# jones-lab-tamu/CBAS

Measured on AMD Instinct MI355X. Metric: frames/sec DINOv3-B/16 224px encode+LSTM classify, 1/2/4/8 MI355X, higher is better.
Workload: dtype f16; 1 GPU; DINOv3 ViT-B/16 66624-frame synthetic 224x224 RGB clip per GPU, batch=64, chunked encode + BiLSTM head (C=9, seq_len=31); batch=64, batches_in_flight=2, frames_per_gpu=66624, parallelism=clip-per-gpu x1, weights=synthetic (seeded counter-based generator), operands=fp16 MFMA, fp32 accumulate/residual; head fp32

## Files before the change

cbas_amd/csrc/gemm_epilogue.h:

```cpp
#pragma once
#include "kernels.h"

__device__ __forceinline__ f32x4 rope_rot(f32x4 a, f32x4 c, f32x4 b, f32x4 s) {
    f32x4 t;
    {
#pragma clang fp contract(off)
        t = b * s;
    }
    return __builtin_elementwise_fma(a, c, t);
}

typedef float f32x2 __attribute__((ext_vector_type(2)));
constexpr int LN_BLOCK = 256;
__device__ __forceinline__ float row16_sum(float v) {
    v += dpp_f32<0xB1>(v);
    v += dpp_f32<0x4E>(v);
    v += dpp_f32<0x141>(v);
    v += dpp_f32<0x140>(v);
    return v;
}
template <int NB>
__device__ __forceinline__ f32x2 ln_pool(const f32x2 (&b)[NB], int nb, float n) {
    float s = 0.f, q = 0.f;
#pragma unroll
    for (int k = 0; k < NB; ++k)
        if (k < nb) { s += b[k][0]; q += b[k][1]; }
    const float mean = s / ((float)nb * n);
    float between = 0.f;
#pragma unroll
    for (int k = 0; k < NB; ++k)
        if (k < nb) {
            const float d = b[k][0] * (1.0f / n) - mean;
            between = fmaf(d, d, between);
// ... 49 lines not shown
            const int n = ncol + j * 16;
            const f32x4 bv = *reinterpret_cast<const f32x4*>(p.bias + n);
            const f32x4 lv = *reinterpret_cast<const f32x4*>(p.lambda + n);
            float* xp = p.out_f32 + (size_t)m * p.ldo + n;
            const f32x4 xv = *reinterpret_cast<const f32x4*>(xp);
            *reinterpret_cast<f32x4*>(xp) = (acc[j] + bv) * lv + xv;
        }
    } else if (EPI == EPI_SWIGLU) {
#pragma unroll
        for (int j = 0; j < 2; ++j) {
            const int n = ncol + j * 16;
            const f32x4 gv = swiglu_fast4(acc[j] + *reinterpret_cast<const f32x4*>(p.bias + n),
                                          acc[j + 2] + *reinterpret_cast<const f32x4*>(p.bias + n + 32));
            const f16x4 hv = {(f16)gv[0], (f16)gv[1], (f16)gv[2], (f16)gv[3]};
            *reinterpret_cast<f16x4*>(p.out_f16 + (size_t)m * p.ldo + (head_col0 >> 1) + (lane >> 4) * 4 + j * 16) = hv;
        }
    } else {
#pragma unroll
        for (int j = 0; j < 4; ++j) {
            const int n = ncol + j * 16;
            const f32x4 bv = *reinterpret_cast<const f32x4*>(p.bias + n);
            const f32x4 w = acc[j] + bv;
            const f32x4 gv = gelu_fast4(w);
            const f16x4 hv = {(f16)gv[0], (f16)gv[1], (f16)gv[2], (f16)gv[3]};
            *reinterpret_cast<f16x4*>(p.out_f16 + (size_t)m * p.ldo + n) = hv;
        }
    }
}

#ifndef CBAS_EPI_PASS_SLABS
#define CBAS_EPI_PASS_SLABS 1
#endif
struct NoPrefetch { __device__ __forceinline__ void operator()() const {} };

template <int EPIX, int TM, typename Pre = NoPrefetch>
__device__ __forceinline__ void gemm_epilogue_tile(const GemmParams& p, int row_base, int head_col0, int lane,
                                                   const f32x4 (&acc)[TM][4], char* scratch, Pre pre = Pre(),
                                                   const float* rope_lds = nullptr, f32x2* ln_red = nullptr) {
    constexpr int EPI = epi_base(EPIX);
    constexpr bool LN = EPIX != EPI;
    const int li = lane & 15, g = lane >> 4;
    if (EPI == EPI_PATCH) {
        pre();
#pragma unroll
        for (int i = 0; i < TM; ++i) {
            const int m = row_base + i * 16 + li;
            if (m < p.M) gemm_epilogue_row<EPI_PATCH>(p, m, head_col0, lane, acc[i]);
        }
    } else if (EPI == EPI_RESID) {
        const f32x4 bvt = *reinterpret_cast<const f32x4*>(p.bias + head_col0 + li * 4);
        const f32x4 lvt = *reinterpret_cast<const f32x4*>(p.lambda + head_col0 + li * 4);
        f32x4 xs[2][4];
        auto load_x = [&](int i, f32x4 (&dst)[4]) {
#pragma unroll
            for (int it = 0; it < 4; ++it) {
                int m = row_base + i * 16 + it * 4 + g;
                m = m < p.M ? m : p.M - 1;
                dst[it] = *reinterpret_cast<const f32x4*>(p.out_f32 + (size_t)m * p.ldo + head_col0 + li * 4);
            }
        };
        load_x(0, xs[0]);
        if (TM > 1) load_x(1, xs[1]);
        pre();
#pragma unroll
        for (int i = 0; i < TM; ++i) {
            char* sc = scratch + (i & 1) * 4096;
#pragma unroll
            for (int j = 0; j < 4; ++j) {
                const int q = (4 * j + g) ^ li;
                *reinterpret_cast<f32x4*>(sc + li * 256 + q * 16) = acc[i][j];
            }
            asm volatile("" ::: "memory");
            uint2 h16r[4];
#pragma unroll
            for (int it = 0; it < 4; ++it) {
                const int r = it * 4 + g;
                const f32x4 y = *reinterpret_cast<const f32x4*>(sc + r * 256 + ((li ^ r) << 4));
                const int m = row_base + i * 16 + r;
                const f32x4 xn = (y + bvt) * lvt + xs[i & 1][it];
                if (m < p.M) *reinterpret_cast<f32x4*>(p.out_f32 + (size_t)m * p.ldo + head_col0 + li * 4) = xn;
                if (LN) {
                    const float bs = row16_sum((xn[0] + xn[1]) + (xn[2] + xn[3]));
                    const f32x4 d = xn - bs * (1.0f / 64.0f);
                    const float bq = row16_sum((d[0] * d[0] + d[1] * d[1]) + (d[2] * d[2] + d[3] * d[3]));
                    if (li == 0) ln_red[(i * 16 + r) * 4] = f32x2{bs, bq};
                    const f32x4 c = __builtin_elementwise_max(__builtin_elementwise_min(xn, f32x4{65504.f, 65504.f, 65504.f, 65504.f}),
                                                              f32x4{-65504.f, -65504.f, -65504.f, -65504.f});
                    union { f16x4 h; uint2 u; } cv;
                    cv.h = f16x4{(f16)c[0], (f16)c[1], (f16)c[2], (f16)c[3]};
                    h16r[it] = cv.u;
                }
            }
            if (LN) {
                const bool odd = li & 1;
#pragma unroll
                for (int it = 0; it < 4; it += 2) {
                    const uint2 send = odd ? h16r[it] : h16r[it + 1];
                    uint2 recv;
                    recv.x = (unsigned)__builtin_amdgcn_update_dpp(0, (int)send.x, 0xB1, 0xf, 0xf, true);
                    recv.y = (unsigned)__builtin_amdgcn_update_dpp(0, (int)send.y, 0xB1, 0xf, 0xf, true);
                    const uint2 own = odd ? h16r[it + 1] : h16r[it];
                    const uint4 outv = odd ? uint4{recv.x, recv.y, own.x, own.y} : uint4{own.x, own.y, recv.x, recv.y};
                    const int m = row_base + i * 16 + (it + (odd ? 1 : 0)) * 4 + g;
                    if (m < p.M) *reinterpret_cast<uint4*>(p.x16_out + (size_t)m * p.N + head_col0 + (li & ~1) * 4) = outv;
                }
            }
            if (i + 2 < TM) load_x(i + 2, xs[i & 1]);
            asm volatile("" ::: "memory");
        }
    } else if (EPI == EPI_GELU_F8) {
        f32x4 bv[4];
#pragma unroll
        for (int j = 0; j < 4; ++j) bv[j] = *reinterpret_cast<const f32x4*>(p.bias + head_col0 + j * 16 + g * 4);
        pre();
        uint8_t* const sc_bytes = reinterpret_cast<uint8_t*>(p.out_sc) + (size_t)(head_col0 >> 7) * p.sc_ldo * 4 + ((head_col0 & 127) >> 5);
#pragma unroll
        for (int half = 0; half < (TM + 3) / 4; ++half) {
#pragma unroll
            for (int ii = 0; ii < 4; ++ii) {
                const int i = half * 4 + ii;
                if (i >= TM) break;
                f32x4 v[4];
#pragma unroll
                for (int j = 0; j < 4; ++j) {
                    const f32x4 w = acc[i][j] + bv[j];
                    v[j] = gelu_fast4(w);
                    if (EPIX == EPI_GELU_F8_H) {
                        const f16x4 hv = {(f16)v[j][0], (f16)v[j][1], (f16)v[j][2], (f16)v[j][3]};
                        v[j] = f32x4{(float)hv[0], (float)hv[1], (float)hv[2], (float)hv[3]};
                    }
                }
                int sb[2];
#pragma unroll
                for (int b = 0; b < 2; ++b) {
                    float a = 0.f;
#pragma unroll
                    for (int e = 0; e < 4; ++e) a = fmaxf(a, fmaxf(fabsf(v[2 * b][e]), fabsf(v[2 * b + 1][e])));
                    a = xor16_max(a);
                    a = xor32_max(a);
                    sb[b] = mx_scale_byte(a);
                }
// ... 156 lines not shown
```

cbas_amd/csrc/gemm_f16_8ph.hip:

```cpp
#include <stdlib.h>
#include <map>
#include <mutex>
#include <queue>
#include <type_traits>
#include <vector>
#include "gemm_epilogue.h"
#include "vit32_epilogue.h"

namespace {

constexpr int BK = 64;
constexpr int BN = 256;

struct PPGrid {
    int main_blocks;
    int tail_row0;
    int n_tiles;
};

__device__ __forceinline__ f16x8 read_frag8(const char* lds_tile, int off) {
    return *reinterpret_cast<const f16x8*>(lds_tile + off);
}

template <int TA, int TB>
// ... 98 lines not shown
        }
    };

    int a_off[2], b_off[2];
    int sa_off = 0, sb_off = 0;
    auto set_frag_offsets = [&] {
        const int frow = lane & 15, fchunk = lane >> 4;
#pragma unroll
        for (int kk = 0; kk < 2; ++kk) {
            const int sw = ((kk * 4 + fchunk) ^ ((frow >> 1) & 7)) << 4;
            a_off[kk] = (wr * WROWS + frow) * 128 + sw;
            b_off[kk] = A_BYTES + (wc * 64 + frow) * 128 + sw;
        }
        sa_off = (wr * WROWS + frow) * 4 + fchunk;
        sb_off = 1024 + (wc * 64 + frow) * 4 + fchunk;
    };

    constexpr bool LNC = EPI == EPI_QKV_LN || EPI == EPI_GELU_LN;
    f32x2 lnp[4];
    auto load_lnp = [&] {
        if constexpr (LNC) {
            if (tid < BM) {
                int m = row0 + tid;
                m = m < p.M ? m : p.M - 1;
                const f32x2* src = reinterpret_cast<const f32x2*>(p.ln_in) + m;
#pragma unroll
                for (int k = 0; k < 4; ++k)
                    if (k < p.ln_parts) lnp[k] = src[(size_t)k * p.ln_ld];
            }
        }
    };

    f32x4 acc[TM][4];
    unsigned long long t_start = 0, t_top = 0, t_pro = 0, t_loop = 0, r_pro = 0, r_loop = 0;
    if (p.stamps) t_start = __builtin_amdgcn_s_memtime();
    load_lnp();
    stage(0, 0, 0); stage(0, 0, 1); stage(0, 0, 2); stage(0, 0, 3);

    struct Frag { f16x8 h[2]; i32x8 v; int sc; };
    Frag a[TMAX], b0[2], b1[2];

#define CBAS_SEG_BARRIER()                      \
    do {                                        \
        __builtin_amdgcn_sched_barrier(0);      \
        __builtin_amdgcn_s_barrier();           \
        __builtin_amdgcn_sched_barrier(0);      \
    } while (0)

    auto mfma_quadrant = [&](auto ha_c, Frag (&bf)[2], int hb) {
        constexpr int ha = decltype(ha_c)::value;
        constexpr int T = ha ? TB : TA, I0 = ha ? TA : 0;
        asm volatile("s_waitcnt lgkmcnt(0)" ::: "memory");
        __builtin_amdgcn_sched_barrier(0);
        __builtin_amdgcn_s_setprio(1);
        if constexpr (F8) {
#pragma unroll
            for (int i = 0; i < T; ++i)
#pragma unroll
                for (int j = 0; j < 2; ++j)
                    acc[I0 + i][hb * 2 + j] = __builtin_amdgcn_mfma_scale_f32_16x16x128_f8f6f4(
                        bf[j].v, a[i].v, acc[I0 + i][hb * 2 + j], 0, 0, 0, bf[j].sc, 0, a[i].sc);
#pragma unroll
            for (int i = 0; i < T; ++i)
#pragma unroll
                for (int j = 0; j < 2; ++j) asm volatile("" : "+v"(acc[I0 + i][hb * 2 + j]));
        } else if constexpr (SPLIT) {
// ... 12 lines not shown
                for (int i = 0; i < T; ++i)
#pragma unroll
                    for (int j = 0; j < 2; ++j)
                        acc[I0 + i][hb * 2 + j] =
                            __builtin_amdgcn_mfma_f32_16x16x32_f16(bf[j].h[kk], a[i].h[kk], acc[I0 + i][hb * 2 + j], 0, 0, 0);
        }
        __builtin_amdgcn_s_setprio(0);
    };
    auto read_frag = [&](Frag& f, const char* buf, int off0, int off1, const char* scb, int sc_off) {
        if constexpr (F8) {
            const i32x4 lo = *reinterpret_cast<const i32x4*>(buf + off0), hi = *reinterpret_cast<const i32x4*>(buf + off1);
            f.v = __builtin_shufflevector(lo, hi, 0, 1, 2, 3, 4, 5, 6, 7);
            asm volatile("ds_read_u8 %0, %1" : "=v"(f.sc) : "v"((unsigned)(uintptr_t)LDS_PTR(scb + sc_off)));
        } else {
            f.h[0] = read_frag8(buf, off0);
            f.h[1] = read_frag8(buf, off1);
        }
    };
    auto read_a = [&](const char* buf, const char* scb, auto h_c) {
        constexpr int h = decltype(h_c)::value;
        constexpr int T = h ? TB : TA, I0 = h ? TA : 0;
#pragma unroll
        for (int i = 0; i < T; ++i)
            read_frag(a[i], buf, a_off[0] + (I0 + i) * 2048, a_off[1] + (I0 + i) * 2048, scb, sa_off + (I0 + i) * 64);
    };
    auto read_b = [&](const char* buf, const char* scb, int h, Frag (&bf)[2]) {
#pragma unroll
        for (int j = 0; j < 2; ++j)
            read_frag(bf[j], buf, b_off[0] + (h * 2 + j) * 2048, b_off[1] + (h * 2 + j) * 2048, scb, sb_off + (h * 2 + j) * 64);
    };
    using H0 = std::integral_constant<int, 0>;
    using H1 = std::integral_constant<int, 1>;

    auto ktile = [&](int b, int t) {
        const char* buf = smem + b * BUF_BYTES;
        const char* scb = sc_lds + b * 2048;
        read_b(buf, scb, 0, b0);
        __builtin_amdgcn_sched_barrier(0);
        read_a(buf, scb, H0{});
        if (t + 1 < nk) stage(b ^ 1, t + 1, 3);
        if (TA == 4) { if (F8) asm volatile("s_waitcnt lgkmcnt(12)" ::: "memory"); else asm volatile("s_waitcnt lgkmcnt(8)" ::: "memory"); }
        else if (TA == 3) { if (F8) asm volatile("s_waitcnt lgkmcnt(9)" ::: "memory"); else asm volatile("s_waitcnt lgkmcnt(6)" ::: "memory"); }
        else { if (F8) asm volatile("s_waitcnt lgkmcnt(6)" ::: "memory"); else asm volatile("s_waitcnt lgkmcnt(4)" ::: "memory"); }
        CBAS_SEG_BARRIER();
        mfma_quadrant(H0{}, b0, 0);
        CBAS_SEG_BARRIER();
        read_b(buf, scb, 1, b1);
        if (t + 2 < nk) stage(b, t + 2, 0);
        CBAS_SEG_BARRIER();
        mfma_quadrant(H0{}, b1, 1);
        CBAS_SEG_BARRIER();
        read_a(buf, scb, H1{});
        if (t + 2 < nk) stage(b, t + 2, 1);
        CBAS_SEG_BARRIER();
        mfma_quadrant(H1{}, b1, 1);
        CBAS_SEG_BARRIER();
        if (t + 2 < nk) {
            stage(b, t + 2, 2);
            asm volatile("s_waitcnt vmcnt(6)" ::: "memory");
        } else {
            asm volatile("s_waitcnt vmcnt(0)" ::: "memory");
        }
        CBAS_SEG_BARRIER();
        mfma_quadrant(H1{}, b0, 0);
        CBAS_SEG_BARRIER();
    };

    for (int id = first;;) {
        if (p.stamps) t_top = __builtin_amdgcn_s_memtime();
        asm volatile("" : "+v"(lane));
        set_tile(id);
        set_frag_offsets();
#pragma unroll
        for (int i = 0; i < TM; ++i)
#pragma unroll
            for (int j = 0; j < 4; ++j) acc[i][j] = f32x4{0.f, 0.f, 0.f, 0.f};
        stage(1, 1, 0); stage(1, 1, 1); stage(1, 1, 2);
        asm volatile("s_waitcnt vmcnt(6)" ::: "memory");
        __builtin_amdgcn_s_barrier();
        if constexpr (LNC) {
            if (tid < BM) {
                const f32x2 st = ln_pool<4>(lnp, p.ln_parts, (float)LN_BLOCK);
                const float inv_d = 1.0f / (float)(p.ln_parts * LN_BLOCK);
                reinterpret_cast<f32x2*>(ln_lds)[tid] = f32x2{st[0] * inv_d, 1.0f / sqrtf(st[1] * inv_d + p.ln_eps)};
            }
        }
        if (p.stamps) { t_pro = __builtin_amdgcn_s_memtime(); r_pro = __builtin_amdgcn_s_memrealtime(); }
        if (wr == 1) __builtin_amdgcn_s_barrier();

        for (int t = 0; t < nk; t += 2) {
            ktile(0, t);
            ktile(1, t + 1);
        }
        if (wr == 0) __builtin_amdgcn_s_barrier();

        if (p.stamps) { t_loop = __builtin_amdgcn_s_memtime(); r_loop = __builtin_amdgcn_s_memrealtime(); }
        const int erow = row0 + wr * WROWS, ecol = col0 + wc * 64;
        const int next = id + stride;
        const bool has_next = next < n_kind;
        asm volatile("" : "+v"(lane));
        if (has_next) set_tile(next);
        if constexpr (SPLIT) {
            vit32_epilogue_tile<EPI, TM>(sp, erow, ecol, lane, acc, smem + BUF_BYTES + wave * 8192, [&] {
                if (has_next) { stage(0, 0, 0); stage(0, 0, 1); stage(0, 0, 2); stage(0, 0, 3); }
            }, rope_lds);
        } else
        gemm_epilogue_tile<EPI, TM>(p, erow, ecol, lane, acc, smem + BUF_BYTES + wave * 8192, [&] {
            if (has_next) { load_lnp(); stage(0, 0, 0); stage(0, 0, 1); stage(0, 0, 2); stage(0, 0, 3); }
        }, rope_lds, EPI == EPI_RESID_LN ? reinterpret_cast<f32x2*>(ln_lds) + (wr * WROWS) * 4 + wc
                                         : reinterpret_cast<f32x2*>(ln_lds) + wr * WROWS);
        if constexpr (EPI == EPI_RESID_LN) {
            asm volatile("s_waitcnt lgkmcnt(0)" ::: "memory");
            __builtin_amdgcn_s_barrier();
            if (tid < BM) {
                const f32x2* e = reinterpret_cast<const f32x2*>(ln_lds) + tid * 4;
                const f32x2 blk[4] = {e[0], e[1], e[2], e[3]};
                const int m = erow - wr * WROWS + tid;
                if (m < p.M) reinterpret_cast<f32x2*>(p.ln_out)[(size_t)((ecol - wc * 64) / LN_BLOCK) * p.ln_ld + m] = ln_pool<4>(blk, 4, 64.0f);
            }
        }
        if (p.stamps && id == first && tid == 0) {
            asm volatile("s_waitcnt vmcnt(0)" ::: "memory");
            unsigned long long* o = p.stamps + (size_t)blockIdx.x * 4;
            o[0] = t_start; o[1] = t_pro; o[2] = t_loop; o[3] = __builtin_amdgcn_s_memtime();
            p.stamps[(size_t)GEMM_STAMP_BLOCKS * 4 + blockIdx.x] = r_loop - r_pro;
        }
        if (p.stamps && id != first && !has_next && tid == 0) {
            unsigned long long* o = p.stamps + (size_t)GEMM_STAMP_BLOCKS * 5 + (size_t)blockIdx.x * 4;
            o[0] = t_top; o[1] = t_pro; o[2] = t_loop; o[3] = __builtin_amdgcn_s_memtime();
        }
        if (!has_next) break;
        id = next;
        if constexpr (EPI != EPI_RESID_LN) {
            asm volatile("s_waitcnt lgkmcnt(0)" ::: "memory");
            __builtin_amdgcn_s_barrier();
        }
    }
#undef CBAS_SEG_BARRIER
}

template <int EPI, int TA, int TB, int TAIL, bool F8>
__global__ __launch_bounds__(512, 2) void gemm_f16_8ph_kernel(GemmParams p, PPGrid g) {
    extern __shared__ __attribute__((aligned(16))) char smem[];
// ... 272 lines not shown
```

cbas_amd/csrc/vit_kernels.hip:

```cpp
#include <stdlib.h>
#include "kernels.h"

namespace {

__global__ void im2col_u8_kernel(const uint8_t* __restrict__ frames, int n, int height, int width,
                                 int64_t frame_stride, int64_t row_stride, int64_t pixel_stride,
                                 f16* __restrict__ A, int nh, int nw, int ps) {
    const int64_t gid = (int64_t)blockIdx.x * blockDim.x + threadIdx.x;
    const int64_t total = (int64_t)n * nh * ps * nw;
    if (gid >= total) return;
    const int px = gid % nw;
    const int64_t t1 = gid / nw;
    const int y = t1 % (nh * ps);
    const int b = t1 / (nh * ps);
    const int py = y / ps, i = y - py * ps;
    const uint8_t* src = frames + b * frame_stride + (int64_t)y * row_stride + (int64_t)px * ps * pixel_stride;
    f16x8 lo, hi;
#pragma unroll
    for (int j = 0; j < 8; ++j) {
        lo[j] = (f16)(float)src[j * pixel_stride];
        hi[j] = (j + 8 < ps) ? (f16)(float)src[(j + 8) * pixel_stride] : (f16)0.f;
    }
    f16* dst = A + ((int64_t)b * nh * nw + (int64_t)py * nw + px) * 256 + i * 16;
    *reinterpret_cast<f16x8*>(dst) = lo;
    *reinterpret_cast<f16x8*>(dst + 8) = hi;
}

__global__ void im2col_f32_kernel(const float* __restrict__ frames, int n, int height, int width,
                                  f16* __restrict__ A, int nh, int nw, int ps) {
    const int64_t gid = (int64_t)blockIdx.x * blockDim.x + threadIdx.x;
    const int64_t total = (int64_t)n * nh * ps * nw;
    if (gid >= total) return;
// ... 203 lines not shown
}

__device__ __forceinline__ int k_off(int row, int chunk) { return row * 128 + ((chunk ^ ((row >> 1) & 7)) << 4); }
__device__ __forceinline__ int v_off(int row, int col) {
    return row * 128 + ((((col >> 4) ^ ((row >> 1) & 3))) << 5) + ((col & 15) << 1);
}

__device__ __forceinline__ void attn_store_f8(const f32x4 (&o)[4], float inv, uint8_t* out8, uint32_t* out_sc, int sc_ld,
                                              size_t row, bool valid, int D, int hd, int g) {
    int sb[2];
#pragma unroll
    for (int b = 0; b < 2; ++b) {
        float a = 0.f;
#pragma unroll
        for (int dt = 2 * b; dt < 2 * b + 2; ++dt)
#pragma unroll
            for (int r = 0; r < 4; ++r) a = fmaxf(a, fabsf(o[dt][r] * inv));
        a = xor16_max(a);
        a = xor32_max(a);
        sb[b] = mx_scale_byte(a);
    }
    if (!valid) return;
    uint8_t* orow = out8 + row * D + hd * 64 + 4 * g;
#pragma unroll
    for (int dt = 0; dt < 4; ++dt) {
        const float m = inv * mx_inv_scale(sb[dt >> 1]);
        *reinterpret_cast<unsigned*>(orow + 16 * dt) = cvt4_e4m3(o[dt][0] * m, o[dt][1] * m, o[dt][2] * m, o[dt][3] * m);
    }
    if (g == 0)
        *reinterpret_cast<uint16_t*>(reinterpret_cast<uint8_t*>(out_sc) + ((size_t)(hd >> 1) * sc_ld + row) * 4 + (hd & 1) * 2) =
            (uint16_t)(sb[0] | (sb[1] << 8));
}

template <int NKT, int NV, int SPLIT>
#ifndef CBAS_ATTN_MIN_WAVES
#define CBAS_ATTN_MIN_WAVES 4
#endif
__global__ __launch_bounds__(SPLIT == 2 ? 256 : 512, (SPLIT == 2 ? (NKT > 14 ? 2 : 3) : (NKT > 14 ? 2 : CBAS_ATTN_MIN_WAVES)))
void attention_kernel(const f16* __restrict__ qkv, const f16* __restrict__ q_cls, void* __restrict__ out_v,
                      uint32_t* __restrict__ out_sc, int sc_ld, int T, int D, int n_heads, int n_pairs) {
    f16* __restrict__ out = reinterpret_cast<f16*>(out_v);
    extern __shared__ __attribute__((aligned(16))) char smem[];
    constexpr int NQK = NV ? NV : NKT;
    constexpr int NG = NV ? (NV + 1) / 2 : NKT / 2;
    constexpr int ROWS = NQK * 16;
    char* Vs = smem;
    char* Ks = smem + ROWS * 128;

    const int tid = threadIdx.x, lane = tid & 63, wave = tid >> 6, nwaves = blockDim.x >> 6;
    int pair = blockIdx.x, half = 0;
    if (SPLIT == 2) {
        pair = ((int)blockIdx.x >> 4) * 8 + ((int)blockIdx.x & 7);
        half = ((int)blockIdx.x >> 3) & 1;
        if (pair >= n_pairs) return;
    }
    const int b = pair / n_heads, hd = pair - b * n_heads;
    const size_t ld = (size_t)3 * D;
    const f16* qbase = qkv + (size_t)b * T * ld + hd * 64;
    const f16* kbase = qbase + D;
    const f16* vbase = qbase + 2 * D;
    const int g = lane >> 4, li = lane & 15;
    const int nq = q_cls ? 1 : T;
    const f16* qsrc = q_cls ? q_cls + (size_t)b * D + hd * 64 : qbase;
    const size_t qld = q_cls ? 0 : ld;
    const int nqt_all = (nq + 15) >> 4;
    const int q_per = SPLIT == 2 ? (nqt_all + 1) / 2 : nqt_all;
    const int qt0 = half * q_per;
    const int nqt = qt0 + q_per < nqt_all ? qt0 + q_per : nqt_all;

    auto load_q = [&](int qt, f16x8 (&qf)[2]) {
        const int q = qt * 16 + li;
        const int qrow = q < nq ? q : nq - 1;
        qf[0] = *reinterpret_cast<const f16x8*>(qsrc + (size_t)qrow * qld + g * 8);
        qf[1] = *reinterpret_cast<const f16x8*>(qsrc + (size_t)qrow * qld + 32 + g * 8);
    };
    f16x8 qf[2] = {};
    int qt = qt0 + wave;
    if (qt < nqt) load_q(qt, qf);

    {
        const int pr = lane >> 3, pos = lane & 7;
        for (int p = wave; p < ROWS / 8; p += nwaves) {
            const int r = p * 8 + pr;
            const int rs = r < T ? r : T - 1;
            const int kc = pos ^ ((r >> 1) & 7);
            const int vc = (((pos >> 1) ^ ((r >> 1) & 3)) << 1) | (pos & 1);
            __builtin_amdgcn_global_load_lds(GLB_PTR(kbase + (size_t)rs * ld + kc * 8), LDS_PTR(Ks + p * 1024), 16, 0, 0);
            __builtin_amdgcn_global_load_lds(GLB_PTR(vbase + (size_t)rs * ld + vc * 8), LDS_PTR(Vs + p * 1024), 16, 0, 0);
        }
        asm volatile("s_waitcnt vmcnt(0)" ::: "memory");
        __syncthreads();
    }

    const char* kb0 = Ks + k_off(li, g);
    const char* kb1 = Ks + k_off(li, 4 + g);
    const char* vb[4];
#pragma unroll
    for (int dt = 0; dt < 4; ++dt) vb[dt] = Vs + v_off(4 * g + (li >> 2), 16 * dt + 4 * (li & 3));
    float tail_bias[4];
#pragma unroll
    for (int r = 0; r < 4; ++r) tail_bias[r] = (NV && (NV - 1) * 16 + 4 * g + r >= T) ? -INFINITY : 0.f;

    for (; qt < nqt; qt += nwaves) {
        const int q = qt * 16 + li;

        f32x4 s[NQK];
#pragma unroll
        for (int grp = 0; grp < (NQK + 1) / 2; ++grp) {
#pragma unroll
            for (int u = 0; u < 2; ++u) {
                const int kt = 2 * grp + u;
                if (kt >= NQK) continue;
                f32x4 acc = {0.f, 0.f, 0.f, 0.f};
                if (NV && kt == NV - 1) acc = f32x4{tail_bias[0], tail_bias[1], tail_bias[2], tail_bias[3]};
                acc = __builtin_amdgcn_mfma_f32_16x16x32_f16(*reinterpret_cast<const f16x8*>(kb0 + kt * 2048), qf[0], acc, 0, 0, 0);
                s[kt] = __builtin_amdgcn_mfma_f32_16x16x32_f16(*reinterpret_cast<const f16x8*>(kb1 + kt * 2048), qf[1], acc, 0, 0, 0);
            }
            __builtin_amdgcn_sched_barrier(0);
        }
        if (qt + nwaves < nqt) load_q(qt + nwaves, qf);
        float mx = -INFINITY;
#pragma unroll
        for (int kt = 0; kt < NQK; ++kt) {
            if (!NV) {
#pragma unroll
                for (int r = 0; r < 4; ++r)
                    if (kt * 16 + 4 * g + r >= T) s[kt][r] = -INFINITY;
            }
            mx = max3_raw(mx, s[kt][0], s[kt][1]);
            mx = max3_raw(mx, s[kt][2], s[kt][3]);
        }
        mx = xor16_max(mx);
        mx = xor32_max(mx);
        const float m2 = mx * 1.4426950408889634f;
        float sum = 0.f;
        f16x8 pf[NG];
#pragma unroll
        for (int grp = 0; grp < NG; ++grp) {
            f32x4 e0, e1 = {0.f, 0.f, 0.f, 0.f};
#pragma unroll
            for (int r = 0; r < 4; ++r) {
                e0[r] = __builtin_amdgcn_exp2f(fmaf(s[2 * grp][r], 1.4426950408889634f, -m2));
                if (2 * grp + 1 < NQK) e1[r] = __builtin_amdgcn_exp2f(fmaf(s[2 * grp + 1 < NQK ? 2 * grp + 1 : 0][r], 1.4426950408889634f, -m2));
            }
            sum += ((e0[0] + e0[1]) + (e0[2] + e0[3])) + ((e1[0] + e1[1]) + (e1[2] + e1[3]));
            pf[grp] = f16x8{(f16)e0[0], (f16)e0[1], (f16)e0[2], (f16)e0[3], (f16)e1[0], (f16)e1[1], (f16)e1[2], (f16)e1[3]};
        }
        sum = xor16_add(sum);
        sum = xor32_add(sum);

        f32x4 o[4];
#pragma unroll
        for (int dt = 0; dt < 4; ++dt) o[dt] = f32x4{0.f, 0.f, 0.f, 0.f};
#pragma unroll
        for (int s2 = 0; s2 < NG; ++s2) {
            f16x8 vf[4];
#pragma unroll
            for (int dt = 0; dt < 4; ++dt) {
                const s16x4 lo = __builtin_amdgcn_ds_read_tr16_b64_v4i16(
                    (__attribute__((address_space(3))) s16x4*)(vb[dt] + s2 * 4096));
                const s16x4 hi = __builtin_amdgcn_ds_read_tr16_b64_v4i16(
                    (__attribute__((address_space(3))) s16x4*)(vb[dt] + s2 * 4096 + 2048));
                union { struct { s16x4 a, b; } s; f16x8 v; } u;
                u.s.a = lo; u.s.b = hi;
                vf[dt] = u.v;
            }
#pragma unroll
            for (int dt = 0; dt < 4; ++dt) o[dt] = __builtin_amdgcn_mfma_f32_16x16x32_f16(vf[dt], pf[s2], o[dt], 0, 0, 0);
            __builtin_amdgcn_sched_barrier(0);
        }
        if (out_sc) {
            attn_store_f8(o, 1.0f / sum, reinterpret_cast<uint8_t*>(out_v), out_sc, sc_ld, (size_t)b * T + q, q < nq, D, hd, g);
        } else if (q < nq) {
            const float inv = 1.0f / sum;
            f16* orow = out + (q_cls ? (size_t)b : (size_t)b * T + q) * D + hd * 64 + 4 * g;
#pragma unroll
            for (int dt = 0; dt < 4; ++dt) {
                const f32x4 w = o[dt] * inv;
                f16x4 hv = {(f16)w[0], (f16)w[1], (f16)w[2], (f16)w[3]};
                *reinterpret_cast<f16x4*>(orow + 16 * dt) = hv;
            }
        }
    }
}

__global__ __launch_bounds__(512, 2) void attention_stream_kernel(const f16* __restrict__ qkv, const f16* __restrict__ q_cls,
                                                                  void* __restrict__ out_v, uint32_t* __restrict__ out_sc, int sc_ld,
                                                                  int T, int D, int n_heads) {
    f16* __restrict__ out = reinterpret_cast<f16*>(out_v);
    __shared__ __attribute__((aligned(16))) char smem[2 * 2 * 64 * 128];
    const int tid = threadIdx.x, lane = tid & 63, wave = tid >> 6;
    const int b = blockIdx.x / n_heads, hd = blockIdx.x - b * n_heads;
    const size_t ld = (size_t)3 * D;
    const f16* qbase = qkv + (size_t)b * T * ld + hd * 64;
    const f16* kbase = qbase + D;
    const f16* vbase = qbase + 2 * D;
    const int g = lane >> 4, li = lane & 15;
    const int nkb = (T + 63) >> 6;
    const int q = (blockIdx.y * 8 + wave) * 16 + li;
    const int nq = q_cls ? 1 : T;
    const bool wave_active = (blockIdx.y * 8 + wave) * 16 < nq;
    const int qrow = q < nq ? q : nq - 1;
    const f16* qsrc = q_cls ? q_cls + (size_t)b * D + hd * 64 : qbase + (size_t)qrow * ld;
    f16x8 qf[2];
    qf[0] = *reinterpret_cast<const f16x8*>(qsrc + g * 8);
    qf[1] = *reinterpret_cast<const f16x8*>(qsrc + 32 + g * 8);

    const int sr = tid >> 3, sc = tid & 7;
    auto load_blk = [&](int kb, f16x8& kv, f16x8& vv) {
        const int r = kb * 64 + sr;
        kv = f16x8{0, 0, 0, 0, 0, 0, 0, 0};
        vv = kv;
        if (r < T) {
            kv = *reinterpret_cast<const f16x8*>(kbase + (size_t)r * ld + sc * 8);
            vv = *reinterpret_cast<const f16x8*>(vbase + (size_t)r * ld + sc * 8);
        }
// ... 220 lines not shown
    if (out_sc) {
        if (wave_active) attn_store_f8(o, 1.0f / l, reinterpret_cast<uint8_t*>(out_v), out_sc, sc_ld, (size_t)b * T + q, q < nq, D, hd, g);
    } else if (q < nq) {
        const float inv = 1.0f / l;
        f16* orow = out + (q_cls ? (size_t)b : (size_t)b * T + q) * D + hd * 64 + 4 * g;
#pragma unroll
        for (int dt = 0; dt < 4; ++dt) {
            const f32x4 w = o[dt] * inv;
            f16x4 hv = {(f16)w[0], (f16)w[1], (f16)w[2], (f16)w[3]};
            *reinterpret_cast<f16x4*>(orow + 16 * dt) = hv;
        }
    }
}

template <int NKT, int NV, int SPLIT>
int launch_attention_t(const f16* qkv, const f16* q_cls, void* out, uint32_t* out_sc, int sc_ld, int n, int T, int D, int n_heads,
                       hipStream_t stream) {
    constexpr int lds = (NV ? NV : NKT) * 16 * 128 * 2;
    static bool attr_set = false;
    if (!attr_set) {
        if (hipFuncSetAttribute(reinterpret_cast<const void*>(&attention_kernel<NKT, NV, SPLIT>),
                                hipFuncAttributeMaxDynamicSharedMemorySize, lds) != hipSuccess)
            return -2;
        attr_set = true;
    }
    if (SPLIT == 2) {
        const int pairs = n * n_heads;
        hipLaunchKernelGGL((attention_kernel<NKT, NV, 2>), dim3(((pairs + 7) / 8) * 16), dim3(256), lds, stream, qkv, q_cls, out,
                           out_sc, sc_ld, T, D, n_heads, pairs);
        return hipGetLastError() == hipSuccess ? 0 : -2;
    }
    constexpr int maxw = 8;
    const int nqt = (T + 15) / 16, rounds = (nqt + maxw - 1) / maxw;
    static const int waves_env = [] { const char* e = getenv("CBAS_ATTN_WAVES"); return e ? atoi(e) : 0; }();
    int nwaves = q_cls ? 4 : (nqt + rounds - 1) / rounds;
    if (!q_cls && waves_env > 0 && waves_env <= 8) nwaves = waves_env;
    hipLaunchKernelGGL((attention_kernel<NKT, NV, 1>), dim3(n * n_heads), dim3(64 * nwaves), lds, stream, qkv, q_cls, out, out_sc,
                       sc_ld, T, D, n_heads, n * n_heads);
    return hipGetLastError() == hipSuccess ? 0 : -2;
}

__global__ void convert_f16_kernel(const float* __restrict__ src, f16* __restrict__ hi, f16* __restrict__ lo, int64_t n) {
    const int64_t i = (int64_t)blockIdx.x * blockDim.x + threadIdx.x;
    if (i >= n) return;
    const float v = src[i];
    const f16 h = (f16)v;
    hi[i] = h;
    if (lo) lo[i] = (f16)(v - (float)h);
}

__global__ void interleave_gate_up_kernel(const float* __restrict__ gate, const float* __restrict__ up, float* __restrict__ out,
                                          int64_t n, int K) {
    const int64_t i = (int64_t)blockIdx.x * blockDim.x + threadIdx.x;
    if (i >= n) return;
    const int64_t r = i / K;
    const int k = (int)(i - r * K), in = (int)(r & 63);
    const int64_t src = ((r >> 6) * 32 + (in & 31)) * K + k;
    out[i] = in < 32 ? gate[src] : up[src];
}

__global__ void pack_fp8_weight_kernel(const float* __restrict__ src, uint8_t* __restrict__ w8, uint32_t* __restrict__ sc,
                                       int N, int K, int n_total, int n0) {
    const int64_t gid = (int64_t)blockIdx.x * blockDim.x + threadIdx.x;
    const int kb_per_row = K / 32;
    if (gid >= (int64_t)N * kb_per_row) return;
    const int n = (int)(gid / kb_per_row), kb = (int)(gid - (int64_t)n * kb_per_row);
    const float* p = src + (size_t)n * K + kb * 32;
    f32x4 v[8];
    float a = 0.f;
// ... 93 lines not shown
int launch_layernorm_f8(const float* x, int64_t ldx, const float* gamma, const float* beta, uint8_t* out8,
                        uint32_t* out_sc, int sc_ld, int M, int D, float eps, hipStream_t stream) {
    if (D % 128 || D > 1024) return -1;
    const int nv = (D / 4 + 63) / 64;
    const dim3 grid((M + 3) / 4), block(256);
    switch (nv) {
        case 2: hipLaunchKernelGGL(layernorm_f8_kernel<2>, grid, block, 0, stream, x, ldx, gamma, beta, out8, out_sc, sc_ld, M, D, eps); break;
        case 3: hipLaunchKernelGGL(layernorm_f8_kernel<3>, grid, block, 0, stream, x, ldx, gamma, beta, out8, out_sc, sc_ld, M, D, eps); break;
        case 4: hipLaunchKernelGGL(layernorm_f8_kernel<4>, grid, block, 0, stream, x, ldx, gamma, beta, out8, out_sc, sc_ld, M, D, eps); break;
        default: return -1;
    }
    return CHECK_LAUNCH();
}

int launch_final_norm_cls(const float* x, const float* gamma, const float* beta, float* cls_f32,
                          f16* cls_f16, int n, int T, int D, float eps, hipStream_t stream, unsigned* nonfinite) {
    const int nv = (D / 4 + 63) / 64;
    const dim3 grid((n + 3) / 4), block(256);
    switch (nv) {
        case 1: hipLaunchKernelGGL(final_norm_cls_kernel<1>, grid, block, 0, stream, x, gamma, beta, cls_f32, cls_f16, n, T, D, eps, nonfinite); break;
        case 2: hipLaunchKernelGGL(final_norm_cls_kernel<2>, grid, block, 0, stream, x, gamma, beta, cls_f32, cls_f16, n, T, D, eps, nonfinite); break;
        case 3: hipLaunchKernelGGL(final_norm_cls_kernel<3>, grid, block, 0, stream, x, gamma, beta, cls_f32, cls_f16, n, T, D, eps, nonfinite); break;
        case 4: hipLaunchKernelGGL(final_norm_cls_kernel<4>, grid, block, 0, stream, x, gamma, beta, cls_f32, cls_f16, n, T, D, eps, nonfinite); break;
        case 5: hipLaunchKernelGGL(final_norm_cls_kernel<5>, grid, block, 0, stream, x, gamma, beta, cls_f32, cls_f16, n, T, D, eps, nonfinite); break;
        default: return -1;
    }
    return CHECK_LAUNCH();
}

int launch_attention(const f16* qkv, const f16* q_cls, void* out, uint32_t* out_sc, int sc_ld, int n, int T, int D, int n_heads,
                     hipStream_t stream) {
    if (q_cls && out_sc) return -1;
    const int nkt = (T + 15) / 16;
    static const int split_env = [] { const char* e = getenv("CBAS_ATTN_SPLIT"); return e ? atoi(e) : 1; }();
    const bool split = split_env == 2 && !q_cls;
    if (nkt == 13) return split ? launch_attention_t<14, 13, 2>(qkv, q_cls, out, out_sc, sc_ld, n, T, D, n_heads, stream)
                                : launch_attention_t<14, 13, 1>(qkv, q_cls, out, out_sc, sc_ld, n, T, D, n_heads, stream);
    if (nkt == 17) return split ? launch_attention_t<18, 17, 2>(qkv, q_cls, out, out_sc, sc_ld, n, T, D, n_heads, stream)
                                : launch_attention_t<18, 17, 1>(qkv, q_cls, out, out_sc, sc_ld, n, T, D, n_heads, stream);
    if (nkt <= 2) return launch_attention_t<2, 0, 1>(qkv, q_cls, out, out_sc, sc_ld, n, T, D, n_heads, stream);
    if (nkt <= 6) return launch_attention_t<6, 0, 1>(qkv, q_cls, out, out_sc, sc_ld, n, T, D, n_heads, stream);
    if (nkt <= 14) return launch_attention_t<14, 0, 1>(qkv, q_cls, out, out_sc, sc_ld, n, T, D, n_heads, stream);
    if (nkt <= 18) return launch_attention_t<18, 0, 1>(qkv, q_cls, out, out_sc, sc_ld, n, T, D, n_heads, stream);
    const int nqb = q_cls ? 1 : ((T + 15) / 16 + 7) / 8;
    static const int stream_env = [] { const char* e = getenv("CBAS_ATTN_STREAM"); return e ? atoi(e) : 3; }();
    if (stream_env == 2) {
        hipLaunchKernelGGL((attention_stream2_kernel<8, false>), dim3(n * n_heads, nqb), dim3(512), 0, stream, qkv, q_cls, out, out_sc, sc_ld, T, D,
                           n_heads);
        return hipGetLastError() == hipSuccess ? 0 : -2;
    }
    if (stream_env == 4) {
        hipLaunchKernelGGL((attention_stream2_kernel<4, true>), dim3(n * n_heads, nqb), dim3(512), 0, stream, qkv, q_cls, out, out_sc, sc_ld, T, D,
                           n_heads);
        return hipGetLastError() == hipSuccess ? 0 : -2;
    }
    if (stream_env == 3) {
        hipLaunchKernelGGL((attention_stream2_kernel<4, false>), dim3(n * n_heads, nqb), dim3(512), 0, stream, qkv, q_cls, out, out_sc, sc_ld, T, D,
                           n_heads);
        return hipGetLastError() == hipSuccess ? 0 : -2;
    }
    hipLaunchKernelGGL(attention_stream_kernel, dim3(n * n_heads, nqb), dim3(512), 0, stream, qkv, q_cls, out, out_sc, sc_ld, T, D, n_heads);
    return hipGetLastError() == hipSuccess ? 0 : -2;
}

int launch_interleave_gate_up(const float* gate, const float* up, float* out, int64_t F, int K, hipStream_t stream) {
    if (F <= 0 || F % 32 || K <= 0) return -1;
    const int64_t n = 2 * F * K;
    hipLaunchKernelGGL(interleave_gate_up_kernel, dim3((unsigned)((n + 255) / 256)), dim3(256), 0, stream, gate, up, out, n, K);
// ... 21 lines not shown
```

Measured before the change: 22940 frames/s.

## Prefetch residual rows into the final GEMM k-tiles through a fetch ring

For residual epilogues, the residual activation rows, bias and lambda vectors are now loaded during the last two k-tiles of the main MFMA loop. These loads take the place of the now-unneeded next-tile staging slots, and their vmcnt waits are tuned to match. A ResidFetch ring whose depth is chosen from TM, and reduced for LN or fp8 variants, holds the prefetched rows, so the epilogue no longer waits on global loads before it starts. The loop peels its final two iterations, and the residual fetch depth is now configurable. The cost is higher VGPR pressure from holding more rows, which could lower occupancy or cause spills.

```diff
diff --git a/cbas_amd/csrc/gemm_epilogue.h b/cbas_amd/csrc/gemm_epilogue.h
--- a/cbas_amd/csrc/gemm_epilogue.h
+++ b/cbas_amd/csrc/gemm_epilogue.h
@@ -1,4 +1,5 @@
 #pragma once
+#include <type_traits>
 #include "kernels.h"
 
 __device__ __forceinline__ f32x4 rope_rot(f32x4 a, f32x4 c, f32x4 b, f32x4 s) {
@@ -114,11 +115,56 @@
 #define CBAS_EPI_PASS_SLABS 1
 #endif
 struct NoPrefetch { __device__ __forceinline__ void operator()() const {} };
-
-template <int EPIX, int TM, typename Pre = NoPrefetch>
+template <int I0, int N, typename F>
+__device__ __forceinline__ void epi_static_for(F&& f) {
+    if constexpr (I0 < N) {
+        f(std::integral_constant<int, I0>{});
+        epi_static_for<I0 + 1, N>(f);
+    }
+}
+
+template <int TM, int DEPTH>
+struct ResidFetch {
+    static_assert(DEPTH >= 1 && DEPTH <= TM + 1, "ring depth");
+    f32x4 xs[DEPTH][4];
+    f32x4 bvt, lvt;
+    const char* xbase;
+    int rlast;
+    unsigned ldo4;
+    __device__ __forceinline__ void init(const GemmParams& p, int row_base, int head_col0) {
+        const int r0 = row_base < p.M ? row_base : p.M - 1;
+        xbase = reinterpret_cast<const char*>(p.out_f32 + (size_t)r0 * p.ldo + head_col0);
+        rlast = p.M - 1 - r0;
+        ldo4 = (unsigned)p.ldo * 4u;
+    }
+    __device__ __forceinline__ void vectors(const GemmParams& p, int head_col0, int lane) {
+        bvt = *reinterpret_cast<const f32x4*>(p.bias + head_col0 + (lane & 15) * 4);
+        lvt = *reinterpret_cast<const f32x4*>(p.lambda + head_col0 + (lane & 15) * 4);
+    }
+    template <int slab>
+    __device__ __forceinline__ void issue(int lane) {
+        const int li = lane & 15, g = lane >> 4;
+#pragma unroll
+        for (int it = 0; it < 4; ++it) {
+            int r = slab * 16 + it * 4 + g;
+            r = r < rlast ? r : rlast;
+            xs[slab % DEPTH][it] = *reinterpret_cast<const f32x4*>(xbase + ((unsigned)r * ldo4 + (unsigned)li * 16u));
+        }
+    }
+};
+#ifndef CBAS_RESID_FETCH_DEPTH
+#define CBAS_RESID_FETCH_DEPTH 8
+#endif
+constexpr int resid_fetch_depth(int tm, bool tight) {
+    const int d = tm > 6 || (tm > 5 && tight) ? 0 : tm > 5 ? 2 : tm == 5 && tight ? 4 : tm;
+    return d < CBAS_RESID_FETCH_DEPTH ? d : CBAS_RESID_FETCH_DEPTH;
+}
+
+template <int EPIX, int TM, typename Pre = NoPrefetch, int XD = 2>
 __device__ __forceinline__ void gemm_epilogue_tile(const GemmParams& p, int row_base, int head_col0, int lane,
                                                    const f32x4 (&acc)[TM][4], char* scratch, Pre pre = Pre(),
-                                                   const float* rope_lds = nullptr, f32x2* ln_red = nullptr) {
+                                                   const float* rope_lds = nullptr, f32x2* ln_red = nullptr,
+                                                   ResidFetch<TM, XD>* held = nullptr) {
     constexpr int EPI = epi_base(EPIX);
     constexpr bool LN = EPIX != EPI;
     const int li = lane & 15, g = lane >> 4;
@@ -130,22 +176,11 @@
             if (m < p.M) gemm_epilogue_row<EPI_PATCH>(p, m, head_col0, lane, acc[i]);
         }
     } else if (EPI == EPI_RESID) {
-        const f32x4 bvt = *reinterpret_cast<const f32x4*>(p.bias + head_col0 + li * 4);
-        const f32x4 lvt = *reinterpret_cast<const f32x4*>(p.lambda + head_col0 + li * 4);
-        f32x4 xs[2][4];
-        auto load_x = [&](int i, f32x4 (&dst)[4]) {
-#pragma unroll
-            for (int it = 0; it < 4; ++it) {
-                int m = row_base + i * 16 + it * 4 + g;
-                m = m < p.M ? m : p.M - 1;
-                dst[it] = *reinterpret_cast<const f32x4*>(p.out_f32 + (size_t)m * p.ldo + head_col0 + li * 4);
-            }
-        };
-        load_x(0, xs[0]);
-        if (TM > 1) load_x(1, xs[1]);
+        auto consume = [&](ResidFetch<TM, XD>& xf) __attribute__((always_inline)) {
         pre();
-#pragma unroll
-        for (int i = 0; i < TM; ++i) {
+        const f32x4 bvt = xf.bvt, lvt = xf.lvt;
+        epi_static_for<0, TM>([&](auto i_c) __attribute__((always_inline)) {
+            constexpr int i = decltype(i_c)::value;
             char* sc = scratch + (i & 1) * 4096;
 #pragma unroll
             for (int j = 0; j < 4; ++j) {
@@ -159,7 +194,7 @@
                 const int r = it * 4 + g;
                 const f32x4 y = *reinterpret_cast<const f32x4*>(sc + r * 256 + ((li ^ r) << 4));
                 const int m = row_base + i * 16 + r;
-                const f32x4 xn = (y + bvt) * lvt + xs[i & 1][it];
+                const f32x4 xn = (y + bvt) * lvt + xf.xs[i % XD][it];
                 if (m < p.M) *reinterpret_cast<f32x4*>(p.out_f32 + (size_t)m * p.ldo + head_col0 + li * 4) = xn;
                 if (LN) {
                     const float bs = row16_sum((xn[0] + xn[1]) + (xn[2] + xn[3]));
@@ -187,8 +222,18 @@
                     if (m < p.M) *reinterpret_cast<uint4*>(p.x16_out + (size_t)m * p.N + head_col0 + (li & ~1) * 4) = outv;
                 }
             }
-            if (i + 2 < TM) load_x(i + 2, xs[i & 1]);
-            asm volatile("" ::: "memory");
+            if constexpr (i + XD < TM) xf.template issue<i + XD>(lane);
+            asm volatile("" ::: "memory");
+        });
+        };
+        if (held) {
+            consume(*held);
+        } else {
+            ResidFetch<TM, XD> own;
+            own.init(p, row_base, head_col0);
+            own.vectors(p, head_col0, lane);
+            epi_static_for<0, (XD < TM ? XD : TM)>([&](auto i_c) __attribute__((always_inline)) { own.template issue<decltype(i_c)::value>(lane); });
+            consume(own);
         }
     } else if (EPI == EPI_GELU_F8) {
         f32x4 bv[4];
diff --git a/cbas_amd/csrc/gemm_f16_8ph.hip b/cbas_amd/csrc/gemm_f16_8ph.hip
--- a/cbas_amd/csrc/gemm_f16_8ph.hip
+++ b/cbas_amd/csrc/gemm_f16_8ph.hip
@@ -154,6 +154,19 @@
     };
 
     f32x4 acc[TM][4];
+    constexpr int XD0 = resid_fetch_depth(TM, F8 || EPI != epi_base(EPI));
+    constexpr bool XPF = epi_base(EPI) == EPI_RESID && !SPLIT && XD0 > 0;
+    constexpr int XD = XPF ? XD0 : 2;
+    ResidFetch<TM, XD> xf;
+    constexpr int X_PRE = XPF ? 2 + 4 * (XD < 3 ? XD : 3) : 0;
+    static_assert(X_PRE <= 63, "vmcnt is a 6-bit count");
+    auto x_slot = [&](auto s_c) {
+        constexpr int s = decltype(s_c)::value;
+        if constexpr (XPF) {
+            if constexpr (s == 0) xf.vectors(p, col0 + wc * 64, lane);
+            if constexpr (s < XD) xf.template issue<s>(lane);
+        }
+    };
     unsigned long long t_start = 0, t_top = 0, t_pro = 0, t_loop = 0, r_pro = 0, r_loop = 0;
     if (p.stamps) t_start = __builtin_amdgcn_s_memtime();
     load_lnp();
@@ -232,13 +245,15 @@
     using H0 = std::integral_constant<int, 0>;
     using H1 = std::integral_constant<int, 1>;
 
-    auto ktile = [&](int b, int t) {
+    auto ktile = [&](auto b_c, int t, auto mode_c) {
+        constexpr int b = decltype(b_c)::value, MODE = decltype(mode_c)::value;
         const char* buf = smem + b * BUF_BYTES;
         const char* scb = sc_lds + b * 2048;
         read_b(buf, scb, 0, b0);
         __builtin_amdgcn_sched_barrier(0);
         read_a(buf, scb, H0{});
-        if (t + 1 < nk) stage(b ^ 1, t + 1, 3);
+        if constexpr (MODE == 2 && b == 1) x_slot(std::integral_constant<int, 3>{});
+        else if (MODE != 0 || t + 1 < nk) stage(b ^ 1, t + 1, 3);
         if (TA == 4) { if (F8) asm volatile("s_waitcnt lgkmcnt(12)" ::: "memory"); else asm volatile("s_waitcnt lgkmcnt(8)" ::: "memory"); }
         else if (TA == 3) { if (F8) asm volatile("s_waitcnt lgkmcnt(9)" ::: "memory"); else asm volatile("s_waitcnt lgkmcnt(6)" ::: "memory"); }
         else { if (F8) asm volatile("s_waitcnt lgkmcnt(6)" ::: "memory"); else asm volatile("s_waitcnt lgkmcnt(4)" ::: "memory"); }
@@ -246,16 +261,21 @@
         mfma_quadrant(H0{}, b0, 0);
         CBAS_SEG_BARRIER();
         read_b(buf, scb, 1, b1);
-        if (t + 2 < nk) stage(b, t + 2, 0);
+        if constexpr (MODE == 2) x_slot(std::integral_constant<int, b * 4>{});
+        else if (MODE == 1 || t + 2 < nk) stage(b, t + 2, 0);
         CBAS_SEG_BARRIER();
         mfma_quadrant(H0{}, b1, 1);
         CBAS_SEG_BARRIER();
         read_a(buf, scb, H1{});
-        if (t + 2 < nk) stage(b, t + 2, 1);
+        if constexpr (MODE == 2) x_slot(std::integral_constant<int, b * 4 + 1>{});
+        else if (MODE == 1 || t + 2 < nk) stage(b, t + 2, 1);
         CBAS_SEG_BARRIER();
         mfma_quadrant(H1{}, b1, 1);
         CBAS_SEG_BARRIER();
-        if (t + 2 < nk) {
+        if constexpr (MODE == 2) {
+            x_slot(std::integral_constant<int, b * 4 + 2>{});
+            if constexpr (b == 0) asm volatile("s_waitcnt vmcnt(%0)" ::"n"(X_PRE) : "memory");
+        } else if (MODE == 1 || t + 2 < nk) {
             stage(b, t + 2, 2);
             asm volatile("s_waitcnt vmcnt(6)" ::: "memory");
         } else {
@@ -271,6 +291,7 @@
         asm volatile("" : "+v"(lane));
         set_tile(id);
         set_frag_offsets();
+        if constexpr (XPF) xf.init(p, row0 + wr * WROWS, col0 + wc * 64);
 #pragma unroll
         for (int i = 0; i < TM; ++i)
 #pragma unroll
@@ -288,9 +309,18 @@
         if (p.stamps) { t_pro = __builtin_amdgcn_s_memtime(); r_pro = __builtin_amdgcn_s_memrealtime(); }
         if (wr == 1) __builtin_amdgcn_s_barrier();
 
-        for (int t = 0; t < nk; t += 2) {
-            ktile(0, t);
-            ktile(1, t + 1);
+        if constexpr (XPF) {
+            for (int t = 0; t + 2 < nk; t += 2) {
+                ktile(H0{}, t, H1{});
+                ktile(H1{}, t + 1, H1{});
+            }
+            ktile(H0{}, nk - 2, std::integral_constant<int, 2>{});
+            ktile(H1{}, nk - 1, std::integral_constant<int, 2>{});
+        } else {
+            for (int t = 0; t < nk; t += 2) {
+                ktile(H0{}, t, H0{});
+                ktile(H1{}, t + 1, H0{});
+            }
         }
         if (wr == 0) __builtin_amdgcn_s_barrier();
 
@@ -308,7 +338,8 @@
         gemm_epilogue_tile<EPI, TM>(p, erow, ecol, lane, acc, smem + BUF_BYTES + wave * 8192, [&] {
             if (has_next) { load_lnp(); stage(0, 0, 0); stage(0, 0, 1); stage(0, 0, 2); stage(0, 0, 3); }
         }, rope_lds, EPI == EPI_RESID_LN ? reinterpret_cast<f32x2*>(ln_lds) + (wr * WROWS) * 4 + wc
-                                         : reinterpret_cast<f32x2*>(ln_lds) + wr * WROWS);
+                                         : reinterpret_cast<f32x2*>(ln_lds) + wr * WROWS,
+        XPF ? &xf : static_cast<ResidFetch<TM, XD>*>(nullptr));
         if constexpr (EPI == EPI_RESID_LN) {
             asm volatile("s_waitcnt lgkmcnt(0)" ::: "memory");
             __builtin_amdgcn_s_barrier();
```

New measurement: 23000 frames/s (median of 6 runs). About the same (+0.3%).

## Overlap V tile load with first QK^T tile in attention kernel

Applied to the files above, without the earlier changes.

Splits the K and V global-to-LDS loads into separate loops and waits only until the K loads and the first Q loads have landed, leaving the V loads in flight. The first query tile then computes QK^T and softmax before a full vmcnt(0) wait and barrier precede the PV product. Inline-asm Q loads and a counted s_waitcnt make this partial wait possible. The change also adds compile-time ablation switches and replaces the env-var split and wave-count controls with compile-time constants. The hand-counted vmcnt logic is fragile if the compiler reorders or inserts other memory ops.

```diff
diff --git a/cbas_amd/csrc/vit_kernels.hip b/cbas_amd/csrc/vit_kernels.hip
--- a/cbas_amd/csrc/vit_kernels.hip
+++ b/cbas_amd/csrc/vit_kernels.hip
@@ -1,3 +1,4 @@
+#include <type_traits>
 #include <stdlib.h>
 #include "kernels.h"
 
@@ -267,6 +268,27 @@
             (uint16_t)(sb[0] | (sb[1] << 8));
 }
 
+__device__ __forceinline__ void load_q_untracked(const f16* p, f16x8 (&qf)[2]) {
+    asm volatile("global_load_dwordx4 %0, %2, off\n\tglobal_load_dwordx4 %1, %2, off offset:64"
+                 : "=&v"(qf[0]), "=&v"(qf[1]) : "v"(p) : "memory");
+}
+__device__ __forceinline__ void wait_vm_leave(int n, f16x8 (&qf)[2]) {
+#define CBAS_WAIT_VM(N) case N: asm volatile("s_waitcnt vmcnt(" #N ")" : "+v"(qf[0]), "+v"(qf[1]) : : "memory"); break;
+    switch (n) {
+        CBAS_WAIT_VM(1) CBAS_WAIT_VM(2) CBAS_WAIT_VM(3) CBAS_WAIT_VM(4) CBAS_WAIT_VM(5) CBAS_WAIT_VM(6) CBAS_WAIT_VM(7) CBAS_WAIT_VM(8)
+        CBAS_WAIT_VM(9) CBAS_WAIT_VM(10)
+        default: asm volatile("s_waitcnt vmcnt(0)" : "+v"(qf[0]), "+v"(qf[1]) : : "memory"); break;
+    }
+#undef CBAS_WAIT_VM
+}
+
+#ifndef CBAS_ATTN16_ABLATE
+#define CBAS_ATTN16_ABLATE 0
+#endif
+#ifndef CBAS_ATTN16_SPLIT
+#define CBAS_ATTN16_SPLIT 1
+#endif
+
 template <int NKT, int NV, int SPLIT>
 #ifndef CBAS_ATTN_MIN_WAVES
 #define CBAS_ATTN_MIN_WAVES 4
@@ -279,6 +301,7 @@
     constexpr int NQK = NV ? NV : NKT;
     constexpr int NG = NV ? (NV + 1) / 2 : NKT / 2;
     constexpr int ROWS = NQK * 16;
+    constexpr int ABL = CBAS_ATTN16_ABLATE;
     char* Vs = smem;
     char* Ks = smem + ROWS * 128;
 
@@ -311,21 +334,31 @@
     };
     f16x8 qf[2] = {};
     int qt = qt0 + wave;
-    if (qt < nqt) load_q(qt, qf);
-
-    {
+    if (qt < nqt) {
+        const int q = qt * 16 + li;
+        load_q_untracked(qsrc + (size_t)(q < nq ? q : nq - 1) * qld + g * 8, qf);
+    }
+
+    int n_vp = 0;
+    if (!(ABL & 16)) {
         const int pr = lane >> 3, pos = lane & 7;
         for (int p = wave; p < ROWS / 8; p += nwaves) {
             const int r = p * 8 + pr;
             const int rs = r < T ? r : T - 1;
             const int kc = pos ^ ((r >> 1) & 7);
+            __builtin_amdgcn_global_load_lds(GLB_PTR(kbase + (size_t)rs * ld + kc * 8), LDS_PTR(Ks + p * 1024), 16, 0, 0);
+        }
+        for (int p = wave; p < ROWS / 8; p += nwaves) {
+            const int r = p * 8 + pr;
+            const int rs = r < T ? r : T - 1;
             const int vc = (((pos >> 1) ^ ((r >> 1) & 3)) << 1) | (pos & 1);
-            __builtin_amdgcn_global_load_lds(GLB_PTR(kbase + (size_t)rs * ld + kc * 8), LDS_PTR(Ks + p * 1024), 16, 0, 0);
             __builtin_amdgcn_global_load_lds(GLB_PTR(vbase + (size_t)rs * ld + vc * 8), LDS_PTR(Vs + p * 1024), 16, 0, 0);
-        }
-        asm volatile("s_waitcnt vmcnt(0)" ::: "memory");
-        __syncthreads();
-    }
+            ++n_vp;
+        }
+    }
+    wait_vm_leave(__builtin_amdgcn_readfirstlane(n_vp), qf);
+    __builtin_amdgcn_s_barrier();
+    asm volatile("" ::: "memory");
 
     const char* kb0 = Ks + k_off(li, g);
     const char* kb1 = Ks + k_off(li, 4 + g);
@@ -336,7 +369,8 @@
 #pragma unroll
     for (int r = 0; r < 4; ++r) tail_bias[r] = (NV && (NV - 1) * 16 + 4 * g + r >= T) ? -INFINITY : 0.f;
 
-    for (; qt < nqt; qt += nwaves) {
+    auto tile = [&](auto first_tile) {
+        constexpr bool FIRST = decltype(first_tile)::value;
         const int q = qt * 16 + li;
 
         f32x4 s[NQK];
@@ -348,15 +382,20 @@
                 if (kt >= NQK) continue;
                 f32x4 acc = {0.f, 0.f, 0.f, 0.f};
                 if (NV && kt == NV - 1) acc = f32x4{tail_bias[0], tail_bias[1], tail_bias[2], tail_bias[3]};
+                if (ABL & (4 | 8)) {
+                    s[kt] = acc + f32x4{(float)qf[0][0], (float)qf[0][1], (float)qf[1][0], (float)(qf[1][1] + (f16)kt)};
+                    continue;
+                }
                 acc = __builtin_amdgcn_mfma_f32_16x16x32_f16(*reinterpret_cast<const f16x8*>(kb0 + kt * 2048), qf[0], acc, 0, 0, 0);
                 s[kt] = __builtin_amdgcn_mfma_f32_16x16x32_f16(*reinterpret_cast<const f16x8*>(kb1 + kt * 2048), qf[1], acc, 0, 0, 0);
             }
             __builtin_amdgcn_sched_barrier(0);
         }
-        if (qt + nwaves < nqt) load_q(qt + nwaves, qf);
+        const bool more = qt + nwaves < nqt;
+        if (!FIRST && more) load_q(qt + nwaves, qf);
         float mx = -INFINITY;
 #pragma unroll
-        for (int kt = 0; kt < NQK; ++kt) {
+        for (int kt = 0; kt < ((ABL & 8) ? 1 : NQK); ++kt) {
             if (!NV) {
 #pragma unroll
                 for (int r = 0; r < 4; ++r)
@@ -375,20 +414,40 @@
             f32x4 e0, e1 = {0.f, 0.f, 0.f, 0.f};
 #pragma unroll
             for (int r = 0; r < 4; ++r) {
+                if (ABL & (1 | 8)) {
+                    e0[r] = s[2 * grp][r];
+                    if (2 * grp + 1 < NQK) e1[r] = s[2 * grp + 1 < NQK ? 2 * grp + 1 : 0][r];
+                    continue;
+                }
                 e0[r] = __builtin_amdgcn_exp2f(fmaf(s[2 * grp][r], 1.4426950408889634f, -m2));
                 if (2 * grp + 1 < NQK) e1[r] = __builtin_amdgcn_exp2f(fmaf(s[2 * grp + 1 < NQK ? 2 * grp + 1 : 0][r], 1.4426950408889634f, -m2));
             }
+            if (ABL & (1 | 8)) {
+                sum += e0[0] + e1[3] + m2;
+                pf[grp] = f16x8{(f16)e0[0], (f16)0.f, (f16)0.f, (f16)0.f, (f16)0.f, (f16)0.f, (f16)0.f, (f16)e1[3]};
+                continue;
+            }
             sum += ((e0[0] + e0[1]) + (e0[2] + e0[3])) + ((e1[0] + e1[1]) + (e1[2] + e1[3]));
             pf[grp] = f16x8{(f16)e0[0], (f16)e0[1], (f16)e0[2], (f16)e0[3], (f16)e1[0], (f16)e1[1], (f16)e1[2], (f16)e1[3]};
         }
         sum = xor16_add(sum);
         sum = xor32_add(sum);
 
+        if (FIRST) {
+            asm volatile("s_waitcnt vmcnt(0)" ::: "memory");
+            __syncthreads();
+            if (more) load_q(qt + nwaves, qf);
+        }
+
         f32x4 o[4];
 #pragma unroll
         for (int dt = 0; dt < 4; ++dt) o[dt] = f32x4{0.f, 0.f, 0.f, 0.f};
 #pragma unroll
         for (int s2 = 0; s2 < NG; ++s2) {
+            if (ABL & (2 | 8)) {
+                o[s2 & 3][s2 & 1] += (float)pf[s2][0] + (float)pf[s2][7];
+                continue;
+            }
             f16x8 vf[4];
 #pragma unroll
             for (int dt = 0; dt < 4; ++dt) {
@@ -416,7 +475,15 @@
                 *reinterpret_cast<f16x4*>(orow + 16 * dt) = hv;
             }
         }
-    }
+    };
+    if (qt < nqt) {
+        tile(std::true_type{});
+        qt += nwaves;
+    } else {
+        asm volatile("s_waitcnt vmcnt(0)" ::: "memory");
+        __syncthreads();
+    }
+    for (; qt < nqt; qt += nwaves) tile(std::false_type{});
 }
 
 __global__ __launch_bounds__(512, 2) void attention_stream_kernel(const f16* __restrict__ qkv, const f16* __restrict__ q_cls,
@@ -703,9 +770,7 @@
     }
     constexpr int maxw = 8;
     const int nqt = (T + 15) / 16, rounds = (nqt + maxw - 1) / maxw;
-    static const int waves_env = [] { const char* e = getenv("CBAS_ATTN_WAVES"); return e ? atoi(e) : 0; }();
-    int nwaves = q_cls ? 4 : (nqt + rounds - 1) / rounds;
-    if (!q_cls && waves_env > 0 && waves_env <= 8) nwaves = waves_env;
+    const int nwaves = q_cls ? 4 : (nqt + rounds - 1) / rounds;
     hipLaunchKernelGGL((attention_kernel<NKT, NV, 1>), dim3(n * n_heads), dim3(64 * nwaves), lds, stream, qkv, q_cls, out, out_sc,
                        sc_ld, T, D, n_heads, n * n_heads);
     return hipGetLastError() == hipSuccess ? 0 : -2;
@@ -865,8 +930,7 @@
                      hipStream_t stream) {
     if (q_cls && out_sc) return -1;
     const int nkt = (T + 15) / 16;
-    static const int split_env = [] { const char* e = getenv("CBAS_ATTN_SPLIT"); return e ? atoi(e) : 1; }();
-    const bool split = split_env == 2 && !q_cls;
+    const bool split = CBAS_ATTN16_SPLIT == 2 && !q_cls;
     if (nkt == 13) return split ? launch_attention_t<14, 13, 2>(qkv, q_cls, out, out_sc, sc_ld, n, T, D, n_heads, stream)
                                 : launch_attention_t<14, 13, 1>(qkv, q_cls, out, out_sc, sc_ld, n, T, D, n_heads, stream);
     if (nkt == 17) return split ? launch_attention_t<18, 17, 2>(qkv, q_cls, out, out_sc, sc_ld, n, T, D, n_heads, stream)
```

New measurement: 23500 frames/s before, 23480 frames/s after, median of 2. Within noise of the previous version (-0.1%).
